# KevinMathewT/multimodal-propaganda-meme-classification

Measured on AMD Instinct MI355X. Metric: memes/sec (fine-tune step) ViT-B/16+BERT-base bs=32, 1/2/4/8 MI355X, higher is better.
Workload: dtype fp16

## Files before the change

include/memehip.h:

```cpp
#ifndef MEMEHIP_H
#define MEMEHIP_H

#include <stdint.h>

#ifdef __cplusplus
extern "C" {
#endif

typedef enum MhStatus {
    MH_OK = 0,
    MH_EINVAL = 1,
    MH_ESHAPE = 2,
    MH_ELAUNCH = 3
} MhStatus;

typedef void* mh_stream_t;

const char* mh_version(void);
const char* mh_status_str(int status);

#define MH_GEMM_MAX_GROUP 8
#define MH_GEMM_GELU 1
#define MH_GEMM_OUT_F32 2
#define MH_GEMM_ACCUM 4
#define MH_GEMM_QUICK_GELU 8
#define MH_GEMM_DERIV_AUX 16

typedef struct MhGemmProblem {
    const void* A;
    const void* B;
    void* C;
    const float* bias;
    const void* residual;
    void* aux;
    const void* mul;
    float* rowsum;
    int32_t M, N, K;
    int32_t lda, ldb, ldc;
    int32_t flags;
    float alpha;
    const uint32_t* drop_rng;
    float drop_p;
    uint32_t drop_stream;
    const int32_t* rows_dev;
    const int32_t* drop_rows;
    int32_t ksplit;
    int32_t reserved_;
} MhGemmProblem;

int mh_gemm_bf16_grouped(const MhGemmProblem* problems , int n_problems, int a_kmajor,
                         int b_kmajor, mh_stream_t stream);
int mh_gemm_ksplit_for(int K, int want);
int mh_gemm_skinny_eligible(const MhGemmProblem* problems , int n_problems, int a_kmajor, int b_kmajor);
int mh_gemm_set_trace(void* device_buffer);

int mh_layernorm_fwd(const void* x , const float* gamma, const float* beta, void* y ,
                     float* y_f32 , float* mean, float* rstd,
                     int rows, int D, float eps, mh_stream_t stream);
int mh_layernorm_bwd(const void* dy , const void* x , const float* gamma,
                     const float* mean, const float* rstd, const void* dx_add ,
                     void* dx , float* part , int n_part, int rows, int D,
                     void* dx_drop ,
                     const uint32_t* rng, float drop_p, uint32_t drop_stream, mh_stream_t stream);
#define MH_LN_MAX_JOBS 4
typedef struct MhLnFwdJob {
    const void* x; const float* gamma; const float* beta; void* y; float* y_f32; float* mean; float* rstd;
    int32_t rows; float eps;
    const int32_t* rows_dev;
} MhLnFwdJob;
typedef struct MhLnBwdJob {
    const void* dy; const void* x; const float* gamma; const float* mean; const float* rstd;
    const void* dx_add; void* dx; float* part; void* dx_drop; const uint32_t* rng;
    int32_t n_part; int32_t rows; float drop_p; uint32_t drop_stream;
    const int32_t* rows_dev;
    const int32_t* drop_rows;
} MhLnBwdJob;
int mh_layernorm_fwd_grouped(const MhLnFwdJob* jobs, int n_jobs, int D, mh_stream_t stream);
int mh_layernorm_bwd_grouped(const MhLnBwdJob* jobs, int n_jobs, int D, mh_stream_t stream);
#define MH_COLSUM_MAX_JOBS 64
typedef struct MhColsumJob {
    const float* part;
    float* out0;
    float* out1;
} MhColsumJob;
int mh_colsum_partials_f32(const MhColsumJob* jobs , int n_jobs, int n_part, int D,
                           float scale, mh_stream_t stream);

int mh_attn_fwd(const void* qkv, const int64_t* key_mask, void* out, float* lse, int B, int S, int H,
                const uint32_t* rng, float drop_p, uint32_t drop_stream, mh_stream_t stream);
int mh_attn_bwd(const void* qkv, const int64_t* key_mask, const void* out, const void* dout,
                const float* lse, float* delta, void* dqkv, int B, int S, int H, const uint32_t* rng,
                float drop_p, uint32_t drop_stream, mh_stream_t stream);
int mh_attn_fwd_packed(const void* qkv, const int64_t* key_mask, void* out, float* lse, const int32_t* cu,
                       const int32_t* row_map, int B, int S, int H, const uint32_t* rng, float drop_p,
                       uint32_t drop_stream, mh_stream_t stream);
int mh_attn_bwd_packed(const void* qkv, const int64_t* key_mask, const void* out, const void* dout,
                       const float* lse, float* delta, void* dqkv, const int32_t* cu, const int32_t* row_map, int B,
                       int S, int H, const uint32_t* rng, float drop_p, uint32_t drop_stream, mh_stream_t stream);

#define MH_ATTN_MAX_GROUP 2
typedef struct MhAttnProblem {
    const void* qkv; const int64_t* key_mask; void* out; float* lse;
    const void* dout; float* delta; void* dqkv;
    const int32_t* cu; const int32_t* row_map;
    const uint32_t* rng; float drop_p; uint32_t drop_stream;
    int32_t B, S, H; int32_t reserved;
} MhAttnProblem;
int mh_attn_fwd_grouped(const MhAttnProblem* problems , int n, mh_stream_t stream);
int mh_attn_bwd_grouped(const MhAttnProblem* problems , int n, mh_stream_t stream);
int mh_attn_set_onepass(int on);

int mh_pack_plan(const int64_t* mask , int B, int S, int pool_index, int32_t* cu, int32_t* row_map,
                 int32_t* inv_map, int64_t* pmask, int32_t* pool_rows, int32_t* n_rows, mh_stream_t stream);
int mh_pack_rows(const void* src , const int32_t* row_map, const int32_t* n_rows, void* dst,
                 int max_rows, int D, mh_stream_t stream);
int mh_unpack_rows(const void* src , const int32_t* inv_map, void* dst ,
                   int max_rows, int D, mh_stream_t stream);

#define MH_ROWS_MAX_JOBS 8
typedef struct {
    const void* src;
    void* dst;
    const int32_t* idx;
    const int32_t* rows_dev;
    int32_t n, rows, D, stride, offset; int32_t reserved_;
} MhRowsJob;
int mh_rows_gather(const MhRowsJob* jobs , int n_jobs, mh_stream_t stream);
int mh_rows_scatter_zero(const MhRowsJob* jobs , int n_jobs, mh_stream_t stream);

int mh_bert_embed_fwd(const int64_t* ids, const float* word, const float* pos, const float* type0,
                      const float* gamma, const float* beta, void* pre ,
                      void* y , float* mean, float* rstd, int B, int S, int D, int vocab,
                      float eps, const uint32_t* rng, float drop_p, uint32_t drop_stream ,
                      mh_stream_t stream);
int mh_bert_embed_bwd(const int64_t* ids, const void* d_pre , float* dword ,
                      float* dpos , float* dtype0 , int B, int S, int D,
                      int vocab, int64_t pad_id, float scale,
                      uint8_t* row_live ,
                      int32_t* first_pos , int32_t* id_count
                      ,
                      mh_stream_t stream);
int mh_bert_embed_bwd_accum(const int64_t* ids, const void* d_pre , float* dword ,
                            float* dpos , float* dtype0 , int B, int S, int D,
                            int vocab, int64_t pad_id, float scale, uint8_t* row_live, int32_t* first_pos, int32_t* id_count,
                            mh_stream_t stream);
int mh_position_ids_from_input_ids(const int64_t* ids , int32_t* pos_ids, int32_t* pos_inv, int B, int S, int pad_id,
                                   int max_position, mh_stream_t stream);
int mh_bert_embed_fwd_pos(const int64_t* ids, const float* word, const float* pos , const float* type0,
                          const float* gamma, const float* beta, void* pre, void* y, float* mean, float* rstd, int B, int S,
                          int D, int vocab, float eps, const uint32_t* rng, float drop_p, uint32_t drop_stream,
                          const int32_t* pos_ids , int max_position, mh_stream_t stream);
int mh_embed_pos_bwd(const void* d_pre , const int32_t* pos_inv ,
                     float* dpos , float* dtype0 , float* scratch ,
                     int B, int S, int D, int max_position, float scale, mh_stream_t stream);
int mh_image_normalize_u8(const uint8_t* src, float* dst, int B, int H, int W, const float* mean3 ,
                          const float* std3 , mh_stream_t stream);
int mh_image_resample_u8(const uint8_t* arena, const int64_t* src_off, const int32_t* hw, const int32_t* xbounds,
                         const int32_t* xcoef, int KX, const int32_t* ybounds, const int32_t* ycoef, int KY, const uint8_t* flip,
                         const uint8_t* vfirst, uint8_t* tmp, uint8_t* out, int B, int max_h, int max_w, int OH, int OW,
                         mh_stream_t stream);
int mh_image_luma_sum_u8(const uint8_t* img, unsigned long long* sums, int B, int HW, mh_stream_t stream);
int mh_image_jitter_rotate_u8(const uint8_t* in, uint8_t* scratch, uint8_t* out, const void* params, unsigned long long* lsum,
                              int B, int H, int W, mh_stream_t stream);
int mh_image_luma_u8(const uint8_t* arena, const int64_t* src_off, const int32_t* hw, uint8_t* gray, int B, int max_hw,
                     mh_stream_t stream);
int mh_image_resample_l_u8(const uint8_t* gray, const int64_t* src_off, const int32_t* hw, const int32_t* xbounds,
                           const int32_t* xcoef, int KX, const int32_t* ybounds, const int32_t* ycoef, int KY, const uint8_t* flip,
                           const uint8_t* vfirst, uint8_t* tmp, uint8_t* out, int B, int max_h, int max_w, int OH, int OW,
                           mh_stream_t stream);
int mh_image_normalize_l_u8(const uint8_t* src, float* dst, int64_t n, float mean, float std, mh_stream_t stream);
int mh_dropout_apply(void* x, int64_t n, const uint32_t* rng, float p, uint32_t stream_id, mh_stream_t stream);
int mh_dropout_mask_u8(uint8_t* out, int64_t n, const uint32_t* rng, float p, uint32_t stream_id,
                       mh_stream_t stream);
int mh_zero_rows_f32(const int64_t* ids, float* table, int n_ids, int D, int vocab, mh_stream_t stream);

int mh_patchify(const float* image, void* patches, int B, int C, int H, int W, int P, mh_stream_t stream);
int mh_patchify_ld(const float* image, void* patches , int B, int C, int H, int W, int P, int ld,
                   mh_stream_t stream);
int mh_copy2d_u32(const void* src, int ld_src, void* dst, int ld_dst, int rows, int cols, int pad_to, mh_stream_t stream);
int mh_vit_assemble_fwd(const void* proj , const float* cls, const float* pos,
                        void* x , int B, int Np, int D, mh_stream_t stream);
int mh_vit_assemble_bwd(const void* dx , void* dproj ,
                        float* dcls, float* dpos, int B, int Np, int D, float scale, mh_stream_t stream);

typedef struct MhHeadParams {
    const float *Wt, *bt;
    const float *Wi, *bi;
    const float *Wf, *bf_;
    const float *Wo, *bo;
} MhHeadParams;
typedef struct MhHeadGrads {
    float *Wt, *bt, *Wi, *bi, *Wf, *bf_, *Wo, *bo;
} MhHeadGrads;

int mh_head_fwd(const MhHeadParams* p , const float* text_hidden ,
                const float* image_hidden , int text_pool_index, float* pooled
                , float* feat , float* fused ,
                float* logits , int B, int S, int Nt, int Dt, int Di, int P, int C,
                const uint32_t* rng, float drop_p, uint32_t drop_stream ,
                const int32_t* text_rows , mh_stream_t stream);
int mh_head_bwd(const MhHeadParams* p , const MhHeadGrads* g , const float* dlogits,
                const float* pooled, const float* feat, const float* fused, float* dfeat ,
                float* dfused , void* d_text_hidden ,
                void* d_image_hidden , int text_pool_index, int B, int S, int Nt,
                int Dt, int Di, int P, int C, float out_scale, const uint32_t* rng, float drop_p,
                uint32_t drop_stream, const int32_t* text_rows , mh_stream_t stream);
int mh_pool_fwd(const float* text_hidden, const float* image_hidden, int text_pool_index, float* pooled, int B, int S,
                int Nt, int Dt, int Di, const int32_t* text_rows, mh_stream_t stream);
int mh_pool_bwd(const float* d_pooled, void* d_text_hidden, void* d_image_hidden, int text_pool_index, int B, int S,
                int Nt, int Dt, int Di, float out_scale, const int32_t* text_rows, mh_stream_t stream);
#define MH_BN_RELU 1
#define MH_BN_FROZEN_STATS 2
int mh_bn1d_fwd(const float* x, int ldx, const float* gamma, const float* beta, float* running_mean, float* running_var,
                float* y, int ldy, float* save_mean, float* save_rstd, int B, int F, float eps, float momentum,
                int training, int relu, mh_stream_t stream);
int mh_bn1d_bwd(const float* dy, int lddy, const float* x, int ldx, const float* y, int ldy, const float* gamma,
                const float* save_mean, const float* save_rstd, float* dx, int lddx, float* dgamma, float* dbeta, int B,
                int F, int relu, mh_stream_t stream);
int mh_ce_fwd_bwd(const float* logits, const int64_t* labels, float* loss, float* dlogits,
                  int32_t* n_correct, int B, int C, float grad_scale,
                  const float* grad_scale_dev ,
                  mh_stream_t stream);
int mh_focal_fwd_bwd(const float* logits, int ld, const float* targets , float* loss,
                     float* dlogits, int32_t* n_correct, int B, float alpha, float gamma, float grad_scale,
                     const float* grad_scale_dev , mh_stream_t stream);
#define MH_LOSS_MEAN 0
#define MH_LOSS_SUM 1
#define MH_LOSS_NONE 2
int mh_ce_opts_fwd_bwd(const float* logits, const int64_t* labels, const float* class_weight ,
                       float* loss , float* dlogits, int32_t* n_correct, int B, int C,
                       int64_t ignore_index, int has_ignore, float label_smoothing, int reduction, float grad_scale,
                       const float* grad_scale_dev , mh_stream_t stream);
int mh_bce_fwd_bwd(const float* logits, int ld, const float* targets , float pos_weight,
                   float* loss, float* dlogits, int32_t* n_correct, int B, int reduction, float grad_scale,
                   const float* grad_scale_dev , mh_stream_t stream);

#define MH_F32_ACCUM 1
#define MH_F32_TANH 2
#define MH_F32_RELU 4
// ... 229 lines not shown
```

multimodal_propaganda_meme_classification_amd/csrc/layernorm.hip:

```cpp
#include "common.h"
#include <stdlib.h>

namespace {

template <int NCH>
MH_DEV void load_row(const h16* __restrict__ p, int D, int lane, float (&v)[NCH][8]) {
#pragma unroll
    for (int i = 0; i < NCH; ++i) {
        const int c = (lane + 64 * i) * 8;
        if (c < D) {
            Pack8 u;
            u.v = *(const i32x4*)(p + c);
#pragma unroll
            for (int e = 0; e < 8; ++e) v[i][e] = mh_bf2f(u.e[e]);
        } else {
#pragma unroll
            for (int e = 0; e < 8; ++e) v[i][e] = 0.f;
        }
    }
}
template <int NCH>
MH_DEV void load_row_f32(const float* __restrict__ p, int D, int lane, float (&v)[NCH][8]) {
#pragma unroll
    for (int i = 0; i < NCH; ++i) {
// ... 97 lines not shown
#pragma unroll
        for (int i = 0; i < NCH; ++i)
#pragma unroll
            for (int e = 0; e < 8; ++e) v[i][e] = (v[i][e] - mu) * rs * g[i][e] + b[i][e];
        store_row<NCH>(y + (size_t)row * D, D, lane, v);
        if (y32) {
#pragma unroll
            for (int i = 0; i < NCH; ++i) {
                const int c = (lane + 64 * i) * 8;
                if (c < D) {
                    *(f32x4*)(y32 + (size_t)row * D + c) = f32x4{v[i][0], v[i][1], v[i][2], v[i][3]};
                    *(f32x4*)(y32 + (size_t)row * D + c + 4) = f32x4{v[i][4], v[i][5], v[i][6], v[i][7]};
                }
            }
        }
        if (lane == 0) {
            if (mean) mean[row] = mu;
            if (rstd) rstd[row] = rs;
        }
    }
}

struct LnBwdGroup {
    int n;
    int start[MH_LN_MAX_JOBS + 1];
    MhLnBwdJob job[MH_LN_MAX_JOBS];
};

template <int NCH, bool DROP, int NWV>
__global__ __launch_bounds__(NWV * 64) void ln_bwd_kernel(const LnBwdGroup grp, int D) {
    __shared__ float red[NWV][64 * 8];
    int j = 0;
    while (j + 1 < grp.n && (int)blockIdx.x >= grp.start[j + 1]) ++j;
    const MhLnBwdJob& jb = grp.job[j];
    const h16* __restrict__ dy = (const h16*)jb.dy;
    const h16* __restrict__ x = (const h16*)jb.x;
    const float* __restrict__ gamma = jb.gamma;
    const float* __restrict__ mean = jb.mean;
    const float* __restrict__ rstd = jb.rstd;
    const h16* __restrict__ dx_add = (const h16*)jb.dx_add;
    h16* __restrict__ dx = (h16*)jb.dx;
    float* __restrict__ part = jb.part;
    h16* __restrict__ dx_drop = (h16*)jb.dx_drop;
    const int n_part = jb.n_part;
    const int rows = jb.rows_dev ? min(jb.rows, *jb.rows_dev) : jb.rows;
    const int32_t* __restrict__ drop_rows = jb.drop_rows;
    const int blk = (int)blockIdx.x - grp.start[j];
    const int lane = threadIdx.x & 63, wave = __builtin_amdgcn_readfirstlane((int)(threadIdx.x >> 6));
    float g[NCH][8], dg[NCH][8], db[NCH][8];
    load_row_f32<NCH>(gamma, D, lane, g);
#pragma unroll
    for (int i = 0; i < NCH; ++i)
#pragma unroll
        for (int e = 0; e < 8; ++e) { dg[i][e] = 0.f; db[i][e] = 0.f; }
    const float invD = 1.0f / (float)D;
    const bool dropj = DROP && dx_drop != nullptr;
    const DropCtx drop = mh_drop_ctx(dropj ? jb.rng : nullptr, jb.drop_p, jb.drop_stream);
    int row = blk * NWV + wave;
    i32x4 nx[NCH], nd[NCH], na[NCH];
    float nmu = 0.f, nrs = 0.f;
    if (row < rows) {
        load_row_raw<NCH>(x + (size_t)row * D, D, lane, nx);
        load_row_raw<NCH>(dy + (size_t)row * D, D, lane, nd);
        if (dx_add) load_row_raw<NCH>(dx_add + (size_t)row * D, D, lane, na);
        nmu = mean[row];
        nrs = rstd[row];
    }
    for (; row < rows; row += n_part * NWV) {
        float xv[NCH][8], dv[NCH][8], av[NCH][8];
        unpack_row<NCH>(nx, xv);
        unpack_row<NCH>(nd, dv);
        if (dx_add) unpack_row<NCH>(na, av);
        const float mu = nmu, rs = nrs;
        const int nrow = row + n_part * NWV;
        if (nrow < rows) {
            load_row_raw<NCH>(x + (size_t)nrow * D, D, lane, nx);
            load_row_raw<NCH>(dy + (size_t)nrow * D, D, lane, nd);
            if (dx_add) load_row_raw<NCH>(dx_add + (size_t)nrow * D, D, lane, na);
            nmu = mean[nrow];
            nrs = rstd[nrow];
        }
        float c1 = 0.f, c2 = 0.f;
#pragma unroll
        for (int i = 0; i < NCH; ++i) {
            const bool ok = (lane + 64 * i) * 8 < D;
#pragma unroll
            for (int e = 0; e < 8; ++e) {
                const float xh = ok ? (xv[i][e] - mu) * rs : 0.f;
                const float dyg = dv[i][e] * g[i][e];
                xv[i][e] = xh;
                dg[i][e] += dv[i][e] * xh;
                db[i][e] += dv[i][e];
                c1 += dyg;
                c2 += dyg * xh;
            }
        }
        c1 = wave_sum(c1) * invD;
        c2 = wave_sum(c2) * invD;
        if (dx_add) {
#pragma unroll
            for (int i = 0; i < NCH; ++i)
#pragma unroll
                for (int e = 0; e < 8; ++e)
                    dv[i][e] = rs * (dv[i][e] * g[i][e] - c1 - xv[i][e] * c2) + av[i][e];
        } else {
#pragma unroll
            for (int i = 0; i < NCH; ++i)
#pragma unroll
                for (int e = 0; e < 8; ++e) dv[i][e] = rs * (dv[i][e] * g[i][e] - c1 - xv[i][e] * c2);
        }
        store_row<NCH>(dx + (size_t)row * D, D, lane, dv);
        const uint64_t drow = (DROP && drop_rows) ? (uint64_t)drop_rows[row] : (uint64_t)row;
        if (DROP && dropj) {
#pragma unroll
            for (int i = 0; i < NCH; ++i) {
                const int c = (lane + 64 * i) * 8;
#pragma unroll
                for (int e = 0; e < 8; ++e) dv[i][e] *= mh_drop_mul(drop, drow * D + c + e);
            }
            store_row<NCH>(dx_drop + (size_t)row * D, D, lane, dv);
        }
    }
    float* pg = part + (size_t)blk * D;
    float* pb = part + (size_t)n_part * D + (size_t)blk * D;
#pragma unroll
    for (int pass = 0; pass < 2; ++pass) {
#pragma unroll
        for (int i = 0; i < NCH; ++i) {
            __syncthreads();
#pragma unroll
            for (int e = 0; e < 8; ++e) red[wave][lane * 8 + (e ^ ((lane >> 2) & 7))] = pass == 0 ? dg[i][e] : db[i][e];
            __syncthreads();
#pragma unroll
            for (int k = 0; k < 8 / NWV; ++k) {
                const int cidx = threadIdx.x + NWV * 64 * k;
                const int col = (cidx >> 3) * 8 + 64 * 8 * i + (cidx & 7);
                const int sidx = (cidx & ~7) | ((cidx & 7) ^ ((cidx >> 5) & 7));
                if (col < D) {
                    float s = 0.f;
#pragma unroll
                    for (int w = 0; w < NWV; ++w) s += red[w][sidx];
                    (pass == 0 ? pg : pb)[col] = s;
                }
            }
        }
    }
}

struct ColsumJobs {
    int n;
    const float* part[MH_COLSUM_MAX_JOBS];
    float* out0[MH_COLSUM_MAX_JOBS];
    float* out1[MH_COLSUM_MAX_JOBS];
};

__global__ __launch_bounds__(256) void colsum_partials_kernel(const ColsumJobs jobs, int n_part, int D, float scale) {
    __shared__ f32x4 red[4][64];
    const int lane = threadIdx.x & 63, wave = threadIdx.x >> 6;
    const int col = blockIdx.x * 256 + lane * 4;
    const int which = blockIdx.y, job = blockIdx.z;
    float* out = which == 0 ? jobs.out0[job] : jobs.out1[job];
    if (!out) return;
    const float* p = jobs.part[job] + (size_t)which * n_part * D;
    f32x4 s = {0.f, 0.f, 0.f, 0.f};
    if (col < D) {
        for (int i0 = wave; i0 < n_part; i0 += 32) {
            f32x4 v[8];
#pragma unroll
            for (int k = 0; k < 8; ++k) {
                const int i = i0 + 4 * k;
                v[k] = *(const f32x4*)(p + (size_t)min(i, n_part - 1) * D + col);
                if (i >= n_part) v[k] = f32x4{0.f, 0.f, 0.f, 0.f};
            }
            s += (v[0] + v[1]) + (v[2] + v[3]);
            s += (v[4] + v[5]) + (v[6] + v[7]);
        }
    }
    red[wave][lane] = s;
    __syncthreads();
    if (wave == 0 && col < D) {
        const f32x4 t = ((red[0][lane] + red[1][lane]) + (red[2][lane] + red[3][lane])) * scale;
        *(f32x4*)(out + col) = t;
    }
}

}

#define LN_FWD_GO(RPW_)                                                                                 \
    do {                                                                                                \
        const int nch = (D / 8 + 63) / 64;                                                              \
        if (nch <= 1) hipLaunchKernelGGL((ln_fwd_kernel<1, RPW_>), dim3(blocks), dim3(256), 0, s, g, D);       \
        else if (nch <= 2) hipLaunchKernelGGL((ln_fwd_kernel<2, RPW_>), dim3(blocks), dim3(256), 0, s, g, D);  \
        else if (nch <= 4) hipLaunchKernelGGL((ln_fwd_kernel<4, RPW_>), dim3(blocks), dim3(256), 0, s, g, D);  \
        else hipLaunchKernelGGL((ln_fwd_kernel<8, RPW_>), dim3(blocks), dim3(256), 0, s, g, D);                \
    } while (0)

extern "C" int mh_layernorm_fwd_grouped(const MhLnFwdJob* jobs, int n_jobs, int D, mh_stream_t stream) {
    if (!jobs || n_jobs < 1 || n_jobs > MH_LN_MAX_JOBS) return MH_EINVAL;
    if (D < 8 || (D % 8) || D > 4096) return MH_ESHAPE;
    static int rpw = -1;
    if (rpw < 0) {
        const char* e = getenv("MEMEHIP_LN_FWD_RPW");
        rpw = (e && atoi(e) == 4) ? 4 : 2;
    }
    const int use_rpw = (rpw == 4 && D <= 1024) ? 4 : 2;
    LnFwdGroup g;
    g.n = n_jobs;
    int blocks = 0;
    for (int i = 0; i < n_jobs; ++i) {
        const MhLnFwdJob& jb = jobs[i];
        if (!jb.x || !jb.gamma || !jb.beta || !jb.y) return MH_EINVAL;
        if (jb.rows < 1) return MH_ESHAPE;
        g.job[i] = jb;
        g.start[i] = blocks;
        blocks += (jb.rows + 4 * use_rpw - 1) / (4 * use_rpw);
    }
    for (int i = n_jobs; i <= MH_LN_MAX_JOBS; ++i) g.start[i] = blocks;
    hipStream_t s = (hipStream_t)stream;
    if (use_rpw == 4) LN_FWD_GO(4);
    else LN_FWD_GO(2);
    return mh_launch_status();
}

extern "C" int mh_layernorm_fwd(const void* x, const float* gamma, const float* beta, void* y, float* y_f32,
                                float* mean, float* rstd, int rows, int D, float eps, mh_stream_t stream) {
    MhLnFwdJob jb = {x, gamma, beta, y, y_f32, mean, rstd, rows, eps, nullptr};
    return mh_layernorm_fwd_grouped(&jb, 1, D, stream);
}

extern "C" int mh_layernorm_bwd_grouped(const MhLnBwdJob* jobs, int n_jobs, int D, mh_stream_t stream) {
    if (!jobs || n_jobs < 1 || n_jobs > MH_LN_MAX_JOBS) return MH_EINVAL;
    if (D < 8 || (D % 8) || D > 2048) return MH_ESHAPE;
    LnBwdGroup g;
    g.n = n_jobs;
    int blocks = 0;
    bool dr = false;
    for (int i = 0; i < n_jobs; ++i) {
        const MhLnBwdJob& jb = jobs[i];
        if (!jb.dy || !jb.x || !jb.gamma || !jb.mean || !jb.rstd || !jb.dx || !jb.part) return MH_EINVAL;
        if (jb.rows < 1 || jb.n_part < 1) return MH_ESHAPE;
        if (jb.dx_drop && !(jb.rng && jb.drop_p > 0.f)) return MH_EINVAL;
        dr = dr || jb.dx_drop != nullptr;
        g.job[i] = jb;
        g.start[i] = blocks;
        blocks += jb.n_part;
    }
    for (int i = n_jobs; i <= MH_LN_MAX_JOBS; ++i) g.start[i] = blocks;
    hipStream_t s = (hipStream_t)stream;
    const int nch = (D / 8 + 63) / 64;
    static int nwv = -1;
    if (nwv < 0) {
        const char* e = getenv("MEMEHIP_LN_BWD_WAVES");
        nwv = (e && atoi(e) == 8) ? 8 : 4;
    }
#define LN_BWD_ARGS dim3(blocks), dim3(nwv * 64), 0, s, g, D
#define LN_BWD_GO(NCH_)                                                                                          \
    do {                                                                                                         \
        if (nwv == 8) {                                                                                          \
            if (dr) hipLaunchKernelGGL((ln_bwd_kernel<NCH_, true, 8>), LN_BWD_ARGS);                             \
            else hipLaunchKernelGGL((ln_bwd_kernel<NCH_, false, 8>), LN_BWD_ARGS);                               \
        } else {                                                                                                 \
            if (dr) hipLaunchKernelGGL((ln_bwd_kernel<NCH_, true, 4>), LN_BWD_ARGS);                             \
            else hipLaunchKernelGGL((ln_bwd_kernel<NCH_, false, 4>), LN_BWD_ARGS);                               \
        }                                                                                                        \
    } while (0)
    if (nch <= 1) LN_BWD_GO(1);
    else if (nch <= 2) LN_BWD_GO(2);
    else LN_BWD_GO(4);
#undef LN_BWD_GO
#undef LN_BWD_ARGS
    return mh_launch_status();
}

extern "C" int mh_layernorm_bwd(const void* dy, const void* x, const float* gamma, const float* mean,
                                const float* rstd, const void* dx_add, void* dx, float* part, int n_part, int rows,
                                int D, void* dx_drop, const uint32_t* rng, float drop_p, uint32_t drop_stream,
                                mh_stream_t stream) {
    MhLnBwdJob jb = {dy, x, gamma, mean, rstd, dx_add, dx, part, dx_drop, rng, n_part, rows, drop_p, drop_stream,
                     nullptr, nullptr};
    return mh_layernorm_bwd_grouped(&jb, 1, D, stream);
}

extern "C" int mh_colsum_partials_f32(const MhColsumJob* jobs, int n_jobs, int n_part, int D, float scale,
                                      mh_stream_t stream) {
    if (!jobs || n_jobs < 1 || n_jobs > MH_COLSUM_MAX_JOBS) return MH_EINVAL;
    if (n_part < 1 || D < 4 || (D % 4)) return MH_ESHAPE;
    ColsumJobs j;
    j.n = n_jobs;
    for (int i = 0; i < n_jobs; ++i) {
        if (!jobs[i].part) return MH_EINVAL;
        j.part[i] = jobs[i].part;
        j.out0[i] = jobs[i].out0;
        j.out1[i] = jobs[i].out1;
    }
    hipLaunchKernelGGL(colsum_partials_kernel, dim3((D + 255) / 256, 2, n_jobs), dim3(256), 0, (hipStream_t)stream, j,
                       n_part, D, scale);
    return mh_launch_status();
}
```

multimodal_propaganda_meme_classification_amd/engine.py:

```python
from __future__ import annotations

import ctypes as C
from collections import namedtuple
from typing import Callable, Dict, List, NamedTuple, Optional, Tuple

import torch

from . import _lib
from ._lib import (MH_GEMM_ACCUM, MH_GEMM_DERIV_AUX, MH_GEMM_GELU, MH_GEMM_OUT_F32, MH_GEMM_QUICK_GELU, MhAttnProblem, MhColsumJob, MhGemmProblem,
                   MhHeadGrads, MhHeadParams, MhLnBwdJob, MhLnFwdJob, MhRowsJob, MhSpanJob)
from .config import Layout, ModelConfig, check_sequence_length

BF16, F32, I64 = torch.bfloat16, torch.float32, torch.int64
LN_PARTS = 512

LAUNCH, PY, WAIT = "launch", "py", "wait"


class Call(NamedTuple):
    fn: Optional[Callable]
    args: object
    name: str
    tag: str
    work: object
    lane: int
    kind: str = LAUNCH


class Segment:

    def __init__(self, name: str, lib=None):
        self.name = name
        self.lib = lib if lib is not None else _lib.load()
        self.calls: List[Call] = []

    def c(self, fn_name: str, *args, tag: Optional[str] = None, work: float = 0.0, lane: int = 0):
        self.calls.append(Call(getattr(self.lib, fn_name), args, fn_name, tag or fn_name, work, lane))

    def py(self, fn: Callable[[], None]):
        self.calls.append(Call(None, fn, PY, PY, 0.0, 0, PY))

    def wait(self, key: str):
        self.calls.append(Call(None, key, WAIT, WAIT, 0.0, 0, WAIT))

    def run(self, stream: int):
        for fn, args, name, _, _, _, kind in self.calls:
            if fn is None:
                if kind == PY:
                    args()
            else:
                st = fn(*args, stream)
                if st != 0:
                    _lib.check(st, name)

    def run2(self, main: "torch.cuda.Stream", side: Optional["torch.cuda.Stream"], events: Dict[str, "torch.cuda.Event"]):
        mp = main.cuda_stream
        sp = side.cuda_stream if side is not None else mp
        forked1 = False
        for fn, args, name, _, _, lane, kind in self.calls:
            if fn is None:
                if kind == PY:
                    args()
                elif kind == WAIT:
                    if args in events:
                        main.wait_event(events.pop(args))
                continue
            if lane == 1 and side is not None:
                if not forked1:
                    e = torch.cuda.Event()
                    e.record(main)
                    side.wait_event(e)
                    forked1 = True
                st = fn(*args, sp)
            else:
                st = fn(*args, mp)
            if st != 0:
                _lib.check(st, name)
        if forked1:
            d = torch.cuda.Event()
            d.record(side)
            events[self.name] = d

    def run_timed(self, stream: int, tag: str, out: list, dyn_scale: float = 1.0):
        for fn, args, name, t, work, _, kind in self.calls:
            if isinstance(work, tuple):
                work = work[0] + work[1] * dyn_scale
            if fn is None:
                if kind == PY:
                    args()
                continue
            if t == tag:
                e0, e1 = torch.cuda.Event(enable_timing=True), torch.cuda.Event(enable_timing=True)
                e0.record()
                st = fn(*args, stream)
                e1.record()
                out.append((e0, e1, work))
            else:
                st = fn(*args, stream)
            if st != 0:
                _lib.check(st, name)

    def __len__(self):
        return len(self.calls)


def _ptr(t: Optional[torch.Tensor]):
    return None if t is None else t.data_ptr()


class LossOptions(NamedTuple):
    weighted: bool
    ignore_index: Optional[int]
    label_smoothing: float
    reduction: str


class Plan:
    def __init__(self, B: int, S: int, lib=None):
        self.B, self.S = B, S
        self.lib = lib
        self.buf: Dict[str, torch.Tensor] = {}
        self.keep: list = []
        self.fwd = Segment("fwd", lib)
        self.loss = Segment("loss", lib)
        self.bwd: List[Segment] = []
        self.bwd_add: Optional[List[Segment]] = None
        self.build_args: Optional[tuple] = None
        self.bucket_after: Dict[str, Tuple[int, int]] = {}
        self.n_launches = 0
        self.gemm_flops = 0.0
        self.gemm_flops_dyn = 0.0
        self.packed = False
        self.dropout_on = False
        self.features = False
        self.loss_opts = None
        self.last_rows = "all"
        self.gather = None
        self._ln_jobs: Dict[int, list] = {}


class Engine:
    def __init__(self, cfg: ModelConfig, layout: Layout, P: torch.Tensor, G: torch.Tensor, SH: torch.Tensor):
        self.cfg, self.layout = cfg, layout
        self.P, self.G, self.SH = P, G, SH
        self.dev = P.device
        assert P.is_cuda and G.is_cuda and SH.is_cuda, "memehip needs HIP device buffers (no CPU fallback)"
        self.kind = cfg.compute_dtype
        self.T16 = torch.float16 if self.kind == "fp16" else torch.bfloat16
        assert SH.dtype == self.T16
        self.lib = _lib.load(self.kind)
        self.gscale = cfg.stream_scale
        self.pack_text = cfg.pack_text
        self.plans: Dict[Tuple[int, int], Plan] = {}
        self.word_row_live = torch.zeros(cfg.text.vocab_size, dtype=torch.uint8, device=self.dev)
        self.word_first = torch.full((cfg.text.vocab_size,), 0x7fffffff, dtype=torch.int32, device=self.dev)
        self.word_count = torch.zeros(cfg.text.vocab_size, dtype=torch.int32, device=self.dev)
        self.loss_scale = torch.ones(1, dtype=F32, device=self.dev)
        self.loss_opts: Optional[LossOptions] = None
        self.class_weight: Optional[torch.Tensor] = None
        self.small0 = layout.n_shadow
        self.small1 = layout.spec[WORD_TABLE].offset
        self._mirror: Optional[torch.Tensor] = None
# ... 538 lines not shown
            pl.loss.c("mh_ce_fwd_bwd", _ptr(logits), _ptr(labels), _ptr(loss), _ptr(self.dlogits), _ptr(ncorrect), B, Cn,
                      1.0, _ptr(eng.loss_scale))
        else:
            assert not opts.weighted or (eng.class_weight is not None and eng.class_weight.numel() == Cn)
            pl.loss.c("mh_ce_opts_fwd_bwd", _ptr(logits), _ptr(labels), _ptr(eng.class_weight) if opts.weighted else None, _ptr(loss),
                      _ptr(self.dlogits), _ptr(ncorrect), B, Cn, opts.ignore_index or 0, int(opts.ignore_index is not None),
                      opts.label_smoothing, _lib.MH_LOSS_SUM if opts.reduction == "sum" else _lib.MH_LOSS_MEAN, 1.0, _ptr(eng.loss_scale))

    def bwd_head(self):
        eng, pl, B, alloc, t, v = self.eng, self.pl, self.B, self.alloc, self.text, self.image
        P_, Cn = self.cfg.proj, self.cfg.num_classes
        s = self.seg("bwd_head")
        dXf = alloc("i.dXf", (v.out_rows, v.D))
        dfeat, dfused = alloc("h.dfeat", (B, 2 * P_), F32), alloc("h.dfused", (B, P_), F32)
        S_h, Nt_h, pool_h, rows_h = self.head_rows
        if self.zero_fill:
            s.py(t.d_last.zero_)
            s.py(dXf.zero_)
        if pl.features:
            h0 = eng.layout.spec["bert_fc.weight"].offset
            h1 = eng.layout.spec["output_fc.bias"].offset + eng.layout.spec["output_fc.bias"].numel
            if self.accum:
                head_grads = eng.mirror()[h0 - eng.small0:h1 - eng.small0]
                self.acc_spans.append((h0, h1 - h0))
            else:
                head_grads = eng.G[h0:h1]
            s.py(head_grads.zero_)
            if pl.features == "sequence":
                s.c("mh_cast_f32_bf16", _ptr(self.d_seq_t), _ptr(t.d_last), t.T * t.D)
                s.c("mh_cast_f32_bf16", _ptr(self.d_seq_i), _ptr(dXf), v.T * v.D)
            else:
                s.c("mh_pool_bwd", _ptr(self.d_pooled), _ptr(t.d_last), _ptr(dXf), pool_h, B, S_h, Nt_h, t.D, v.D, float(eng.gscale),
                    _ptr(rows_h))
        else:
            hg = self.hg
            if self.accum:
                hg = MhHeadGrads()
                for fld, nm in HEAD_FIELDS:
                    setattr(hg, fld, _ptr(self.g(nm)))
                pl.keep.append(hg)
            s.c("mh_head_bwd", C.byref(self.hp), C.byref(hg), _ptr(self.dlogits), _ptr(self.pooled), _ptr(self.feat),
                _ptr(self.fused), _ptr(dfeat), _ptr(dfused), _ptr(t.d_last), _ptr(dXf), pool_h, B, S_h, Nt_h, t.D, v.D, P_, Cn,
                float(eng.gscale), *self.site(self.p_head, 7), _ptr(rows_h))
        t.grads, v.grads = self._text_grads(), self._image_grads()
        self.t_dpre = alloc("t.dpre", (t.T, t.D))
        self._ln_bwd(s, [
            self._ln_bwd_job(dXf, v.x[v.L], IMG + "layernorm", self.mf, self.rf, v.d_last, v.out_rows, v.D),
            self._text_ln2_bwd(t.L - 1) if t.L >= v.L else None])

    def _text_grads(self) -> List[Grads]:
        t, B, alloc = self.text, self.B, self.alloc
        dh = [alloc(f"t.dh{i}", (t.T, t.I)) for i in range(2)]
        da = [alloc(f"t.da{i}", (t.T, t.D)) for i in range(2)]
        dqkv = [alloc(f"t.dqkv{i}", (t.T, 3 * t.D)) for i in range(2)]
        dam = [alloc(f"t.dam{i}", (t.T, t.D)) for i in range(2)] if t.p_h > 0 else da
        df = [alloc(f"t.df{i}", (t.T, t.D)) for i in range(3)]
        dfm = [alloc(f"t.dfm{i}", (t.T, t.D)) for i in range(3)] if t.p_h > 0 else df
        dy, dctx = alloc("t.dy", (t.T, t.D)), alloc("t.dctx", (t.T, t.D))
        t.delta = alloc("t.delta", (B, t.H, t.S), F32)
        out = [Grads(d_out=dfm[l % 3], dh=dh[l & 1], d_mid=dy, d_proj=dam[l & 1], res=da[l & 1], dctx=dctx, res_full=da[l & 1],
                     dctx_full=dctx, dqkv=dqkv[l & 1], d_in=t.d_x(l - 1), df=df[l % 3]) for l in range(t.L)]
        if t.compact:
            c_df, c_dh, c_dy = alloc("t.dfrows", (B, t.D)), alloc("t.dhrows", (B, t.I)), alloc("t.dyrows", (B, t.D))
            c_da, c_dctx = alloc("t.darows", (B, t.D)), alloc("t.dctxrows", (B, t.D))
            if t.rows(t.L - 1) != t.T:
                out[-1] = out[-1]._replace(d_out=c_df, dh=c_dh, d_mid=c_dy, d_proj=c_da, res=c_da, dctx=c_dctx, df=c_df)
        return out

    def _image_grads(self) -> List[Grads]:
        v, B, alloc = self.image, self.B, self.alloc
        dh = [alloc(f"i.dh{i}", (v.T, v.I)) for i in range(2)]
        dxp = [alloc(f"i.dxp{i}", (v.T, v.D)) for i in range(2)]
        dqkv = [alloc(f"i.dqkv{i}", (v.T, 3 * v.D)) for i in range(2)]
        dw, dctx, du = alloc("i.dw", (v.T, v.D)), alloc("i.dctx", (v.T, v.D)), alloc("i.du", (v.T, v.D))
        v.delta = alloc("i.delta", (B, v.H, v.S), F32)
        out = [Grads(d_out=v.d_x(l), dh=dh[l & 1], d_mid=dw, d_proj=dxp[l & 1], res=dxp[l & 1], dctx=dctx, res_full=dxp[l & 1],
                     dctx_full=dctx, dqkv=dqkv[l & 1], d_in=du) for l in range(v.L)]
        if v.compact:
            c_dh, c_dw = alloc("i.dhrows", (B, v.I)), alloc("i.dwrows", (B, v.D))
            c_dxp, c_dctx = alloc("i.dxprows", (B, v.D)), alloc("i.dctxrows", (B, v.D))
            if v.rows(v.L - 1) != v.T:
                out[-1] = out[-1]._replace(dh=c_dh, d_mid=c_dw, d_proj=c_dxp, res=c_dxp, dctx=c_dctx)
        return out

    def _text_ln2_bwd(self, l) -> Optional[LnBwd]:
        t = self.text
        if not (0 <= l < t.L):
            return None
        a, g = t.acts[l], t.grads[l]
        return self._ln_bwd_job(t.d_x(l), a.f, t.name(l, "output.LayerNorm"), a.m2, a.r2, g.df, a.rows, t.D, dx_drop=g.d_out,
                                drop=self.site(t.p_h, 16 * (l + 1) + 3), **t.live(a.rows, drop=True))

    def _text_embed_ln_bwd(self, s: Segment) -> LnBwd:
        t = self.text
        d_emb = t.d_x(-1)
        if self.pl.packed:
            d_emb = self.alloc("t.dX_dense", (t.T, t.D))
            s.c("mh_unpack_rows", _ptr(t.d_x(-1)), _ptr(self.inv_map), _ptr(d_emb), t.T, t.D)
        if t.p_h > 0:
            s.c("mh_dropout_apply", _ptr(d_emb), t.T * t.D, self.rng.data_ptr(), float(t.p_h), 1)
        return self._ln_bwd_job(d_emb, self.pre0, TXT + "embeddings.LayerNorm", self.m0, self.r0, self.t_dpre, t.T, t.D)

    def bwd_layer(self, l):
        t, v = self.text, self.image
        s = self.seg(f"bwd_layer_{l}")
        s.wait(f"bwd_layer_{l + 2}")
        lay = [(tw, tw.acts[l], tw.roles(l), tw.grads[l], tw.rows(l)) for tw in self.towers if l < tw.L]
        a, ga = (t.acts[l], t.grads[l]) if l < t.L else (None, None)
        b, gb = (v.acts[l], v.grads[l]) if l < v.L else (None, None)
        self._gemm(s, [self._linear_dgrad(tw, l, "output.dense", g.d_out, g.dh, M, tw.D, tw.I, mul=a_.h, deriv_aux=True, quick=tw.quick,
                                          **tw.live(M)) for tw, a_, r, g, M in lay], False, True)
        self._gemm(s, [self._linear_dgrad(tw, l, "intermediate.dense", g.dh, g.d_mid, M, tw.I, tw.D, residual=g.df, **tw.live(M))
                       for tw, a_, r, g, M in lay], False, True)
        self._ln_bwd(s, [
            self._ln_bwd_job(ga.d_mid, a.a, t.name(l, t.ln_mid), a.m1, a.r1, ga.res, a.rows, t.D, dx_drop=ga.d_proj,
                             drop=self.site(t.p_h, 16 * (l + 1) + 2), **t.live(a.rows, drop=True)) if a else None,
            self._ln_bwd_job(gb.d_mid, b.xp, v.name(l, v.ln_mid), b.m2, b.r2, gb.res, b.rows, v.D, dx_add=gb.d_out) if b else None])
        self._gemm(s, [self._linear_dgrad(tw, l, "attention.output.dense", g.d_proj, g.dctx, M, tw.D, tw.D, **tw.live(M))
                       for tw, a_, r, g, M in lay], False, True)
        self._rows(s, [j for tw, a_, r, g, M in lay if M != tw.T
                       for j in (tw.pool._replace(src=g.dctx, dst=g.dctx_full, rows_dev=tw.rows_dev),
                                 tw.pool._replace(src=g.res, dst=g.res_full, rows_dev=tw.rows_dev))], scatter=True)
        self._attn(s, [self._attn_prob(tw, l, dout=g.dctx_full, delta=tw.delta, dqkv=g.dqkv) for tw, a_, r, g, M in reversed(lay)],
                   backward=True)
        self._gemm(s, [self._linear_dgrad(tw, l, tw.attn + "query", g.dqkv, g.d_in, tw.T, 3 * tw.D, tw.D, 3,
                                          residual=g.res_full if tw.post_ln else None, **tw.live(tw.T)) for tw, a_, r, g, M in lay], False, True)
        t_job = self._text_ln2_bwd(l - 1) if l >= 1 else self._text_embed_ln_bwd(s)
        self._ln_bwd(s, [
            t_job,
            self._ln_bwd_job(gb.d_in, v.x[l], v.name(l, "layernorm_before"), b.m1, b.r1, v.d_x(l - 1), v.T, v.D,
                             dx_add=gb.res_full) if b else None])
        for tw, a_, r, g, M in lay:
            self._gemm(s, [
                self._linear_wgrad(tw, l, "output.dense", g.d_out, a_.g, M, tw.D, tw.I, **tw.live(M)),
                self._linear_wgrad(tw, l, "intermediate.dense", g.dh, r.ffn_in, M, tw.I, tw.D, **tw.live(M)),
                self._linear_wgrad(tw, l, "attention.output.dense", g.d_proj, a_.pctx, M, tw.D, tw.D, **tw.live(M)),
                self._linear_wgrad(tw, l, tw.attn + "query", g.dqkv, r.attn_in, tw.T, 3 * tw.D, tw.D, 3, **tw.live(tw.T))],
                True, True, lane=1)
        rng = [r for r in self.eng.layout.layer_ranges if r[0] == l][0]
        self.pl.bucket_after[s.name] = (rng[1], rng[2])

    def bwd_embed(self):
        eng, pl, B, alloc, v, tw = self.eng, self.pl, self.B, self.alloc, self.cfg.image, self.image
        Np, Ti, Di = v.n_patches, tw.T, tw.D
        s = self.seg("bwd_embed")
        i_dproj = alloc("i.dproj", (B * Np, Di))
        d_x0 = tw.d_x(-1)
        if v.pre_ln:
            d_x0 = alloc("i.dx0pre", (Ti, Di))
            self._ln_bwd(s, [self._ln_bwd_job(tw.d_x(-1), pl.buf["i.x0pre"], IMG + "pre_layernorm", pl.buf["i.mpre"], pl.buf["i.rpre"],
                                              d_x0, Ti, Di)])
        s.c("mh_vit_assemble_bwd", _ptr(d_x0), _ptr(i_dproj), _ptr(self.g(IMG + "embeddings.cls_token")),
            _ptr(self.g(IMG + "embeddings.position_embeddings")), B, Np, Di, 1.0 / eng.gscale)
        self._patch_wgrad(s, i_dproj)
        if self.gather_world <= 0:
            self._table_grads(s, self.ids, self.t_dpre, self.prev_ids, B)
        for D, jobs in pl._ln_jobs.items():
            for i0 in range(0, len(jobs), _lib.MH_COLSUM_MAX_JOBS):
                chunk = jobs[i0:i0 + _lib.MH_COLSUM_MAX_JOBS]
                arr = (MhColsumJob * len(chunk))()
                for j, (part, o0, o1) in enumerate(chunk):
                    arr[j].part, arr[j].out0, arr[j].out1 = _ptr(part), _ptr(o0), _ptr(o1)
                pl.keep.append(arr)
                s.c("mh_colsum_partials_f32", arr, len(chunk), LN_PARTS, D, 1.0 / eng.gscale)
        if self.accum:
            self._accum_spans(s)
        tail0 = eng.layout.layer_ranges[-1][2]
        if self.gather_world <= 0:
            pl.bucket_after[s.name] = (tail0, eng.layout.n_total)
        else:
            self._bwd_embed_tables(s, tail0)

    def _patch_wgrad(self, s: Segment, i_dproj):
        eng, pl, alloc, v, Di = self.eng, self.pl, self.alloc, self.cfg.image, self.image.D
        Kp, Kpp, Tp = v.patch_dim, v.patch_dim_padded, self.B * v.n_patches
        gw = gw_out = eng.g(IMG + "embeddings.patch_embeddings.projection.weight")
        gb = self.g(IMG + "embeddings.patch_embeddings.projection.bias") if v.patch_bias else None
        nsplit = min(_lib.MH_GEMM_MAX_GROUP, max(1, Tp // 512))
        plain_add = self.accum and nsplit == 1 and Kpp == Kp
        if self.accum and not plain_add:
            gw = gw_out = alloc("i.dwp_acc", (Di * Kp,), F32)
            self.acc_extra.append((eng.g(IMG + "embeddings.patch_embeddings.projection.weight"), gw_out))
        if Kpp != Kp:
            gw = alloc("i.dwp_pad", (Di * Kpp,), F32)
        if nsplit > 1:
            chunk = -(-Tp // nsplit)
            chunk = -(-chunk // 8) * 8
            part_w = alloc("i.dwp_part", (2, nsplit, Di * Kpp), F32)
            part_b = alloc("i.dbp_part", (2, nsplit, Di), F32)
            probs = []
            for i in range(nsplit):
                k0 = i * chunk
                kk = min(chunk, Tp - k0)
                if kk <= 0:
                    part_w[0, i].zero_(), part_b[0, i].zero_()
                    continue
                probs.append(self._wgrad_prob(i_dproj[k0:], self.patches[k0:], part_w[0, i], part_b[0, i], kk, Di, Kpp))
            self._gemm(s, probs, True, True)
            for part, out, D_ in ((part_w, gw, Di * Kpp), (part_b, gb, Di)):
                if out is None:
                    continue
                arr = (MhColsumJob * 1)()
                arr[0].part, arr[0].out0, arr[0].out1 = _ptr(part), _ptr(out), None
                pl.keep.append(arr)
                s.c("mh_colsum_partials_f32", arr, 1, nsplit, D_, 1.0)
        else:
            self._gemm(s, [self._wgrad_prob(i_dproj, self.patches, gw, gb, Tp, Di, Kpp, accum=plain_add)], True, True)
        if Kpp != Kp:
            s.c("mh_copy2d_u32", _ptr(gw), Kpp, _ptr(gw_out), Kp, Di, Kp, Kp)

    def _table_grads(self, sg: Segment, ids_, dpre_, prev_, nb):
        eng, t, S, Dt = self.eng, self.cfg.text, self.S, self.text.D
        roberta = t.position_scheme == "roberta"
        gword = eng.g(WORD_TABLE)
        gtype0 = self.g(TXT + "embeddings.token_type_embeddings.weight", written=Dt)[:Dt] if t.type_vocab > 0 else None
        gpos = self.g(TXT + "embeddings.position_embeddings.weight", written=None if roberta else S * Dt)
        if not self.accum:
            sg.c("mh_zero_rows_f32", _ptr(prev_), _ptr(gword), nb * S, Dt, t.vocab_size)
        dpos = self.alloc("t.dpos_by_s", (S, Dt), F32) if roberta else gpos
        sg.c("mh_bert_embed_bwd_accum" if self.accum else "mh_bert_embed_bwd", _ptr(ids_), _ptr(dpre_), _ptr(gword), _ptr(dpos), _ptr(gtype0),
             nb, S, Dt, t.vocab_size, int(t.pad_token_id), 1.0 / eng.gscale, eng.word_row_live.data_ptr(), eng.word_first.data_ptr(),
             eng.word_count.data_ptr())
        if roberta:
            pos_inv = self.pos_inv
            if ids_ is not self.ids:
                pos_ids = self.alloc("t.pos_ids_all", (nb, S), torch.int32, zero=True)
                pos_inv = self.alloc("t.pos_inv_all", (nb, t.max_position), torch.int32, zero=True)
                sg.c("mh_position_ids_from_input_ids", _ptr(ids_), _ptr(pos_ids), _ptr(pos_inv), nb, S, int(t.pad_token_id),
                     t.max_position)
            sg.c("mh_embed_pos_bwd", _ptr(dpre_), _ptr(pos_inv), _ptr(gpos), None, None, nb, S, Dt, t.max_position,
                 1.0 / eng.gscale)
        if self.accum:
            window = eng._window_ids
            sg.py(lambda: window.append(ids_.clone()))
        else:
            sg.py(lambda: prev_.copy_(ids_))

    def _bwd_embed_tables(self, s: Segment, tail0: int):
        eng, pl, t, B, S, W, alloc = self.eng, self.pl, self.cfg.text, self.B, self.S, self.gather_world, self.alloc
        Tt, Dt = self.text.T, self.text.D
        first_tbl = TXT + ("embeddings.token_type_embeddings.weight" if t.type_vocab > 0
                           else "embeddings.position_embeddings.weight")
        tbl0 = eng.layout.spec[first_tbl].offset
        assert eng.layout.spec[TXT + "embeddings.word_embeddings.weight"].offset + t.vocab_size * Dt + 3 >= eng.layout.n_total - 3
        pl.bucket_after[s.name] = (tail0, tbl0)
        ids_all = alloc("ids_all", (W * B, S), I64, zero=True)
        prev_all = alloc("prev_ids_all", (W * B, S), I64, zero=True)
        dpre_all = alloc("t.dpre_all", (W * Tt, Dt))
        pl.gather = [(self.ids, ids_all), (self.t_dpre, dpre_all)]
        self._table_grads(self.seg("bwd_embed_tables"), ids_all, dpre_all, prev_all, W * B)
```

Baseline: 3732.

## Merge patch-wgrad and LayerNorm column-sum reductions into one heterogeneous launch

Introduces a per-job column-sum kernel with its own n_part, D and scale, which lets the patch-embedding weight/bias partial reductions and all LayerNorm gamma/beta partial reductions run in a single launch instead of several. The kernel picks the number of column lanes per block from n_part and uses a flattened block index with a binary search over job start offsets. It also prefetches the next row chunk into registers and reduces through shared memory. This is meant to cut launch overhead and raise parallelism on the small reductions. In exchange the kernel is more complex, and the padded-weight copy now has to be deferred until after the merged launch.

Result: no change. 3721 (-0.3%).

```diff
diff --git a/include/memehip.h b/include/memehip.h
--- a/include/memehip.h
+++ b/include/memehip.h
@@ -85,6 +85,13 @@
 } MhColsumJob;
 int mh_colsum_partials_f32(const MhColsumJob* jobs , int n_jobs, int n_part, int D,
                            float scale, mh_stream_t stream);
+typedef struct MhColsumSpec {
+    const float* part;
+    float* out0;
+    float* out1;
+    int32_t n_part; int32_t D; float scale;
+} MhColsumSpec;
+int mh_colsum_jobs_f32(const MhColsumSpec* jobs , int n_jobs, mh_stream_t stream);
 
 int mh_attn_fwd(const void* qkv, const int64_t* key_mask, void* out, float* lse, int B, int S, int H,
                 const uint32_t* rng, float drop_p, uint32_t drop_stream, mh_stream_t stream);
diff --git a/multimodal_propaganda_meme_classification_amd/csrc/layernorm.hip b/multimodal_propaganda_meme_classification_amd/csrc/layernorm.hip
--- a/multimodal_propaganda_meme_classification_amd/csrc/layernorm.hip
+++ b/multimodal_propaganda_meme_classification_amd/csrc/layernorm.hip
@@ -273,36 +273,99 @@
     const float* part[MH_COLSUM_MAX_JOBS];
     float* out0[MH_COLSUM_MAX_JOBS];
     float* out1[MH_COLSUM_MAX_JOBS];
+    int n_part[MH_COLSUM_MAX_JOBS];
+    int D[MH_COLSUM_MAX_JOBS];
+    float scale[MH_COLSUM_MAX_JOBS];
+    int start[MH_COLSUM_MAX_JOBS + 1];
 };
 
-__global__ __launch_bounds__(256) void colsum_partials_kernel(const ColsumJobs jobs, int n_part, int D, float scale) {
-    __shared__ f32x4 red[4][64];
-    const int lane = threadIdx.x & 63, wave = threadIdx.x >> 6;
-    const int col = blockIdx.x * 256 + lane * 4;
-    const int which = blockIdx.y, job = blockIdx.z;
-    float* out = which == 0 ? jobs.out0[job] : jobs.out1[job];
-    if (!out) return;
-    const float* p = jobs.part[job] + (size_t)which * n_part * D;
+constexpr int CS_QUADS = 4;
+
+__host__ __device__ inline int colsum_lanes_log2(int n_part) { return n_part >= 256 ? 4 : n_part >= 128 ? 5 : 6; }
+
+template <int LG>
+MH_DEV void colsum_group(const float* __restrict__ part, float* __restrict__ out, int cg, int n_part, int D, float scale,
+                         f32x4* quad) {
+    constexpr int lanes = 1 << LG, slots = 256 >> LG, chunk_rows = slots * 4 * CS_QUADS;
+    const int tid = threadIdx.x, c = tid & (lanes - 1), r = tid >> LG;
+    const int col = (cg * lanes + c) * 4;
+    const bool okc = col < D;
+    const float* p = part + (okc ? col : 0);
+    f32x4 v[4 * CS_QUADS];
+    auto load = [&](int base) {
+#pragma unroll
+        for (int j = 0; j < CS_QUADS; ++j) {
+            if (base + 4 * slots * j < n_part) {
+                const int q = j * slots + r;
+                const int row0 = base + (q >> 2) * 16 + (q & 3);
+#pragma unroll
+                for (int k = 0; k < 4; ++k)
+                    v[4 * j + k] = *(const f32x4*)(p + (size_t)min(row0 + 4 * k, n_part - 1) * D);
+            } else {
+#pragma unroll
+                for (int k = 0; k < 4; ++k) v[4 * j + k] = f32x4{0.f, 0.f, 0.f, 0.f};
+            }
+        }
+    };
     f32x4 s = {0.f, 0.f, 0.f, 0.f};
-    if (col < D) {
-        for (int i0 = wave; i0 < n_part; i0 += 32) {
-            f32x4 v[8];
-#pragma unroll
-            for (int k = 0; k < 8; ++k) {
-                const int i = i0 + 4 * k;
-                v[k] = *(const f32x4*)(p + (size_t)min(i, n_part - 1) * D + col);
-                if (i >= n_part) v[k] = f32x4{0.f, 0.f, 0.f, 0.f};
-            }
-            s += (v[0] + v[1]) + (v[2] + v[3]);
-            s += (v[4] + v[5]) + (v[6] + v[7]);
-        }
-    }
-    red[wave][lane] = s;
+    load(0);
+    for (int base = 0; base < n_part; base += chunk_rows) {
+#pragma unroll
+        for (int j = 0; j < CS_QUADS; ++j) {
+            const int q = j * slots + r;
+            const int row0 = base + (q >> 2) * 16 + (q & 3);
+#pragma unroll
+            for (int k = 0; k < 4; ++k)
+                if (row0 + 4 * k >= n_part) v[4 * j + k] = f32x4{0.f, 0.f, 0.f, 0.f};
+            const f32x4 qv = (v[4 * j] + v[4 * j + 1]) + (v[4 * j + 2] + v[4 * j + 3]);
+            if constexpr (slots == 4) s += qv;
+            else quad[j * 256 + tid] = qv;
+        }
+        if (base + chunk_rows < n_part) load(base + chunk_rows);
+        if constexpr (slots > 4) {
+            __syncthreads();
+            if (r < 4) {
+#pragma unroll
+                for (int m = 0; m < slots; m += 4) {
+                    f32x4 q[4];
+#pragma unroll
+                    for (int k = 0; k < 4; ++k) q[k] = quad[(m + k) * 4 * lanes + tid];
+#pragma unroll
+                    for (int k = 0; k < 4; ++k) s += q[k];
+                }
+            }
+            __syncthreads();
+        }
+    }
+    if (r < 4) quad[tid] = s;
     __syncthreads();
-    if (wave == 0 && col < D) {
-        const f32x4 t = ((red[0][lane] + red[1][lane]) + (red[2][lane] + red[3][lane])) * scale;
+    if (r == 0 && okc) {
+        const f32x4 t = ((quad[c] + quad[lanes + c]) + (quad[2 * lanes + c] + quad[3 * lanes + c])) * scale;
         *(f32x4*)(out + col) = t;
     }
+}
+
+__global__ __launch_bounds__(256) void colsum_partials_kernel(const ColsumJobs J) {
+    __shared__ f32x4 quad[256 * CS_QUADS];
+    int job = 0;
+#pragma unroll
+    for (int step = MH_COLSUM_MAX_JOBS / 2; step; step >>= 1)
+        if (job + step < J.n && (int)blockIdx.x >= J.start[job + step]) job += step;
+    const int n_part = J.n_part[job], D = J.D[job], lg = colsum_lanes_log2(n_part);
+    const int ncg = (D + (4 << lg) - 1) / (4 << lg);
+    int cg = (int)blockIdx.x - J.start[job];
+    float* out = J.out0[job];
+    int which = 0;
+    if (!out || cg >= ncg) {
+        if (out) cg -= ncg;
+        out = J.out1[job];
+        which = 1;
+    }
+    const float* part = J.part[job] + (size_t)which * n_part * D;
+    const float scale = J.scale[job];
+    if (lg == 4) colsum_group<4>(part, out, cg, n_part, D, scale, quad);
+    else if (lg == 5) colsum_group<5>(part, out, cg, n_part, D, scale, quad);
+    else colsum_group<6>(part, out, cg, n_part, D, scale, quad);
 }
 
 }
@@ -402,19 +465,38 @@
     return mh_layernorm_bwd_grouped(&jb, 1, D, stream);
 }
 
+extern "C" int mh_colsum_jobs_f32(const MhColsumSpec* jobs, int n_jobs, mh_stream_t stream) {
+    if (!jobs || n_jobs < 1 || n_jobs > MH_COLSUM_MAX_JOBS) return MH_EINVAL;
+    ColsumJobs j;
+    j.n = n_jobs;
+    int64_t blocks = 0;
+    for (int i = 0; i < n_jobs; ++i) {
+        const MhColsumSpec& jb = jobs[i];
+        if (!jb.part || ((uintptr_t)jb.part & 15) || (((uintptr_t)jb.out0 | (uintptr_t)jb.out1) & 15)) return MH_EINVAL;
+        if (jb.n_part < 1 || jb.D < 4 || (jb.D % 4)) return MH_ESHAPE;
+        j.part[i] = jb.part;
+        j.out0[i] = jb.out0;
+        j.out1[i] = jb.out1;
+        j.n_part[i] = jb.n_part;
+        j.D[i] = jb.D;
+        j.scale[i] = jb.scale;
+        j.start[i] = (int)blocks;
+        const int cols = 4 << colsum_lanes_log2(jb.n_part);
+        const int ncg = (jb.D + cols - 1) / cols;
+        blocks += (int64_t)ncg * ((jb.out0 ? 1 : 0) + (jb.out1 ? 1 : 0));
+        if (blocks > 0x7fffffff) return MH_ESHAPE;
+    }
+    for (int i = n_jobs; i <= MH_COLSUM_MAX_JOBS; ++i) j.start[i] = (int)blocks;
+    if (blocks == 0) return MH_OK;
+    hipLaunchKernelGGL(colsum_partials_kernel, dim3((unsigned)blocks), dim3(256), 0, (hipStream_t)stream, j);
+    return mh_launch_status();
+}
+
 extern "C" int mh_colsum_partials_f32(const MhColsumJob* jobs, int n_jobs, int n_part, int D, float scale,
                                       mh_stream_t stream) {
     if (!jobs || n_jobs < 1 || n_jobs > MH_COLSUM_MAX_JOBS) return MH_EINVAL;
     if (n_part < 1 || D < 4 || (D % 4)) return MH_ESHAPE;
-    ColsumJobs j;
-    j.n = n_jobs;
-    for (int i = 0; i < n_jobs; ++i) {
-        if (!jobs[i].part) return MH_EINVAL;
-        j.part[i] = jobs[i].part;
-        j.out0[i] = jobs[i].out0;
-        j.out1[i] = jobs[i].out1;
-    }
-    hipLaunchKernelGGL(colsum_partials_kernel, dim3((D + 255) / 256, 2, n_jobs), dim3(256), 0, (hipStream_t)stream, j,
-                       n_part, D, scale);
-    return mh_launch_status();
-}
+    MhColsumSpec spec[MH_COLSUM_MAX_JOBS];
+    for (int i = 0; i < n_jobs; ++i) spec[i] = MhColsumSpec{jobs[i].part, jobs[i].out0, jobs[i].out1, n_part, D, scale};
+    return mh_colsum_jobs_f32(spec, n_jobs, stream);
+}
diff --git a/multimodal_propaganda_meme_classification_amd/engine.py b/multimodal_propaganda_meme_classification_amd/engine.py
--- a/multimodal_propaganda_meme_classification_amd/engine.py
+++ b/multimodal_propaganda_meme_classification_amd/engine.py
@@ -7,7 +7,7 @@
 import torch
 
 from . import _lib
-from ._lib import (MH_GEMM_ACCUM, MH_GEMM_DERIV_AUX, MH_GEMM_GELU, MH_GEMM_OUT_F32, MH_GEMM_QUICK_GELU, MhAttnProblem, MhColsumJob, MhGemmProblem,
+from ._lib import (MH_GEMM_ACCUM, MH_GEMM_DERIV_AUX, MH_GEMM_GELU, MH_GEMM_OUT_F32, MH_GEMM_QUICK_GELU, MhAttnProblem, MhColsumSpec, MhGemmProblem,
                    MhHeadGrads, MhHeadParams, MhLnBwdJob, MhLnFwdJob, MhRowsJob, MhSpanJob)
 from .config import Layout, ModelConfig, check_sequence_length
 
@@ -852,17 +852,12 @@
                                               d_x0, Ti, Di)])
         s.c("mh_vit_assemble_bwd", _ptr(d_x0), _ptr(i_dproj), _ptr(self.g(IMG + "embeddings.cls_token")),
             _ptr(self.g(IMG + "embeddings.position_embeddings")), B, Np, Di, 1.0 / eng.gscale)
-        self._patch_wgrad(s, i_dproj)
+        sums, after = self._patch_wgrad(s, i_dproj)
         if self.gather_world <= 0:
             self._table_grads(s, self.ids, self.t_dpre, self.prev_ids, B)
-        for D, jobs in pl._ln_jobs.items():
-            for i0 in range(0, len(jobs), _lib.MH_COLSUM_MAX_JOBS):
-                chunk = jobs[i0:i0 + _lib.MH_COLSUM_MAX_JOBS]
-                arr = (MhColsumJob * len(chunk))()
-                for j, (part, o0, o1) in enumerate(chunk):
-                    arr[j].part, arr[j].out0, arr[j].out1 = _ptr(part), _ptr(o0), _ptr(o1)
-                pl.keep.append(arr)
-                s.c("mh_colsum_partials_f32", arr, len(chunk), LN_PARTS, D, 1.0 / eng.gscale)
+        self._finish_sums(s, sums)
+        for call in after:
+            s.c(*call)
         if self.accum:
             self._accum_spans(s)
         tail0 = eng.layout.layer_ranges[-1][2]
@@ -897,17 +892,23 @@
                     continue
                 probs.append(self._wgrad_prob(i_dproj[k0:], self.patches[k0:], part_w[0, i], part_b[0, i], kk, Di, Kpp))
             self._gemm(s, probs, True, True)
-            for part, out, D_ in ((part_w, gw, Di * Kpp), (part_b, gb, Di)):
-                if out is None:
-                    continue
-                arr = (MhColsumJob * 1)()
-                arr[0].part, arr[0].out0, arr[0].out1 = _ptr(part), _ptr(out), None
-                pl.keep.append(arr)
-                s.c("mh_colsum_partials_f32", arr, 1, nsplit, D_, 1.0)
+            sums = [(part, out, None, nsplit, D_, 1.0) for part, out, D_ in ((part_w, gw, Di * Kpp), (part_b, gb, Di)) if out is not None]
         else:
             self._gemm(s, [self._wgrad_prob(i_dproj, self.patches, gw, gb, Tp, Di, Kpp, accum=plain_add)], True, True)
-        if Kpp != Kp:
-            s.c("mh_copy2d_u32", _ptr(gw), Kpp, _ptr(gw_out), Kp, Di, Kp, Kp)
+            sums = []
+        return sums, ([("mh_copy2d_u32", _ptr(gw), Kpp, _ptr(gw_out), Kp, Di, Kp, Kp)] if Kpp != Kp else [])
+
+    def _finish_sums(self, s: Segment, sums):
+        eng, pl = self.eng, self.pl
+        sums = sums + [(part, o0, o1, LN_PARTS, D, 1.0 / eng.gscale) for D, jobs in pl._ln_jobs.items() for part, o0, o1 in jobs]
+        for i0 in range(0, len(sums), _lib.MH_COLSUM_MAX_JOBS):
+            chunk = sums[i0:i0 + _lib.MH_COLSUM_MAX_JOBS]
+            arr = (MhColsumSpec * len(chunk))()
+            for j, (part, o0, o1, n_part, D_, scale) in enumerate(chunk):
+                e = arr[j]
+                e.part, e.out0, e.out1, e.n_part, e.D, e.scale = _ptr(part), _ptr(o0), _ptr(o1), n_part, D_, scale
+            pl.keep.append(arr)
+            s.c("mh_colsum_jobs_f32", arr, len(chunk))
 
     def _table_grads(self, sg: Segment, ids_, dpre_, prev_, nb):
         eng, t, S, Dt = self.eng, self.cfg.text, self.S, self.text.D
```
